# ayumiymk/DiG

Hardware: AMD Instinct MI355X
Metric: pretrain images/sec (32x128, 2-view, mask 0.7) ViT-S/4 (higher is better)
Workload: dtype bf16

## Files before the change

### cpu_abi/dig_cpu.cpp

```cpp
#include <algorithm>
#include <cmath>
#include <cstdint>
#include <cstring>
#include <vector>

typedef void* hipStream_t;
#include "../include/dig_block_types.h"
enum { DIG_OK = 0, DIG_ERR_ARG = -1, DIG_ERR_ALIGN = -2, DIG_ERR_LAUNCH = -3, DIG_ERR_UNSUPPORTED = -4 };
typedef uint16_t bf16_t;

struct dig_dropout_t {
  unsigned k0, k1, thr;
  float scale;
  unsigned pk0, pk1, pthr;
  float pscale;
  int rows_per_sample;
};

namespace {

inline float bf2f(bf16_t h) {
  const uint32_t u = (uint32_t)h << 16;
  float f;
  std::memcpy(&f, &u, 4);
// ... 1009 lines not shown
  for (int k = 0; k < 4; ++k) accs4[k] = stats6[(k >> 1) * 3 + 1 + (k & 1)] * acc_scale;
  return DIG_OK;
}
int dig_step_meters(const float* loss, const float* contra, const float* pixel, const float* accs4, const int* counts, int n_counts,
                    const float* grad_norm, float* out10, hipStream_t) {
  if (!loss || !contra || !pixel || !accs4 || !counts || n_counts <= 0 || !out10) return DIG_ERR_ARG;
  int lo = counts[0], hi = counts[0];
  for (int i = 1; i < n_counts; ++i) { lo = std::min(lo, counts[i]); hi = std::max(hi, counts[i]); }
  out10[0] = loss[0]; out10[1] = contra[0]; out10[2] = pixel[0];
  for (int k = 0; k < 4; ++k) out10[3 + k] = accs4[k];
  out10[7] = (float)lo; out10[8] = (float)hi; out10[9] = grad_norm ? grad_norm[0] : NAN;
  return DIG_OK;
}
int dig_ce_rows(float* logits, int n, int m, int label_offset, float gscale, float* out3, hipStream_t) {
  if (!logits || !out3 || n <= 0 || m <= 0 || label_offset < 0 || label_offset + n > m) return DIG_ERR_ARG;
  for (int i = 0; i < n; ++i) {
    float* row = logits + (size_t)i * m;
    const int label = i + label_offset;
    float mx = -3.0e38f;
    for (int j = 0; j < m; ++j) mx = std::max(mx, row[j]);
    const float zl = row[label];
    float s = 0.f;
    int gt = 0;
    for (int j = 0; j < m; ++j) { s += std::exp(row[j] - mx); gt += row[j] > zl; }
    const float lse = mx + std::log(s);
    for (int j = 0; j < m; ++j) row[j] = gscale * (std::exp(row[j] - mx) / s - (j == label ? 1.f : 0.f));
    out3[0] += lse - zl;
    if (gt < 1) out3[1] += 1.f;
    if (gt < 5) out3[2] += 1.f;
  }
  return DIG_OK;
}

static int adamw_core(float* p, const float* g, float* m, float* v, bf16_t* shadow, long long n, const unsigned char* group, float lr0,
                      float wd0, float lr1, float wd1, float beta1, float beta2, float eps, float inv_bc1, float inv_sqrt_bc2,
                      float grad_scale, const float* finite_gate) {
  if (finite_gate && !std::isfinite(finite_gate[0])) return DIG_OK;
#pragma omp parallel for
  for (long long i = 0; i < n; ++i) {
    const int grp = group[i >> 8] & 0x7f;
    if (grp == 2) {
      if (shadow) shadow[i] = f2bf(p[i]);
      continue;
    }
    const float lr = grp ? lr1 : lr0, wd = grp ? wd1 : wd0;
    const float gk = g[i] * grad_scale;
    float P = p[i] * (1.0f - lr * wd);
    const float M = m[i] * beta1 + gk * (1.0f - beta1);
    const float V = v[i] * beta2 + gk * gk * (1.0f - beta2);
    P -= (lr * inv_bc1) * (M / (std::sqrt(V) * inv_sqrt_bc2 + eps));
    p[i] = P; m[i] = M; v[i] = V;
    if (shadow) shadow[i] = f2bf(P);
  }
  return DIG_OK;
}

int dig_adamw_bias_corrections(float beta1, float beta2, int step, float* out2) {
  if (!out2 || step < 1) return DIG_ERR_ARG;
  out2[0] = (float)(1.0 / (1.0 - std::pow((double)beta1, (double)step)));
  out2[1] = (float)(1.0 / std::sqrt(1.0 - std::pow((double)beta2, (double)step)));
  return DIG_OK;
}

struct AdamTrMat { long long off, dst_off; int rows, cols, tile0, pad; };

int dig_adamw_step_tr(float* p, const float* g, float* m, float* v, void* bf16_shadow, long long n, const unsigned char* group_flags, float lr0,
// ... 557 lines not shown
```

### dig_amd/csrc/loss.hip

```cpp
#include "common.h"

namespace {

__global__ void l2norm_fwd_kernel(const float* __restrict__ x, float* __restrict__ y, float* __restrict__ inv_norm, int n, int C,
                                  float eps) {
  const int r = blockIdx.x * (blockDim.x >> 6) + (threadIdx.x >> 6);
  const int lane = threadIdx.x & 63;
  if (r >= n) return;
  float s = 0.f;
  for (int c = lane; c < C; c += 64) { const float v = x[(size_t)r * C + c]; s += v * v; }
  s = wave_sum(s);
  const float inv = 1.0f / fmaxf(sqrtf(s), eps);
  for (int c = lane; c < C; c += 64) y[(size_t)r * C + c] = x[(size_t)r * C + c] * inv;
  if (lane == 0) inv_norm[r] = inv;
}

__global__ void l2norm_bwd_kernel(const float* __restrict__ dy, const float* __restrict__ y, const float* __restrict__ inv_norm,
                                  float* __restrict__ dx, int n, int C) {
  const int r = blockIdx.x * (blockDim.x >> 6) + (threadIdx.x >> 6);
  const int lane = threadIdx.x & 63;
  if (r >= n) return;
  float s = 0.f;
  for (int c = lane; c < C; c += 64) s += y[(size_t)r * C + c] * dy[(size_t)r * C + c];
  s = wave_sum(s);
  const float inv = inv_norm[r];
  for (int c = lane; c < C; c += 64) dx[(size_t)r * C + c] = (dy[(size_t)r * C + c] - y[(size_t)r * C + c] * s) * inv;
}

template <bool TB>
__global__ __launch_bounds__(256) void sgemm_kernel(const float* __restrict__ A, const float* __restrict__ B, float* __restrict__ C,
                                                    int I, int J, int R, int lda, int ldb, int ldc, float alpha, int r_per_split) {
  constexpr int TS = 32, KS = 64;
  __shared__ float As[KS][TS + 1];
// ... 70 lines not shown
      atomicAdd(out, lse - zl);
      if (gt < 0.5f) atomicAdd(out + 1, 1.f);
      if (gt < 4.5f) atomicAdd(out + 2, 1.f);
    }
    return;
  }
  __shared__ float red2[256];
  const float mine[3] = {lse - zl, gt < 0.5f ? 1.f : 0.f, gt < 4.5f ? 1.f : 0.f};
  float tot[3];
  if (dig_grid_sum_last<3>(ws, mine, tot, red2)) { out[0] += tot[0]; out[1] += tot[1]; out[2] += tot[2]; }
}

__global__ void infonce_finish_kernel(const float* __restrict__ stats6, float loss_scale, float acc_scale, float* __restrict__ contra,
                                      float* __restrict__ accs4) {
  if (threadIdx.x == 0) contra[0] = (stats6[0] + stats6[3]) * loss_scale;
  if (threadIdx.x < 4) accs4[threadIdx.x] = stats6[(threadIdx.x >> 1) * 3 + 1 + (threadIdx.x & 1)] * acc_scale;
}

__global__ __launch_bounds__(64) void step_meters_kernel(const float* __restrict__ loss, const float* __restrict__ contra, const float* __restrict__ pixel,
                                                        const float* __restrict__ accs4, const int* __restrict__ counts, int n_counts,
                                                        const float* __restrict__ grad_norm, float* __restrict__ out10) {
  int lo = 0x7fffffff, hi = -0x7fffffff - 1;
  for (int i = threadIdx.x; i < n_counts; i += 64) { const int c = counts[i]; lo = min(lo, c); hi = max(hi, c); }
#pragma unroll
  for (int o = 32; o > 0; o >>= 1) { lo = min(lo, __shfl_xor(lo, o, 64)); hi = max(hi, __shfl_xor(hi, o, 64)); }
  if (threadIdx.x == 0) {
    out10[0] = loss[0]; out10[1] = contra[0]; out10[2] = pixel[0];
    out10[7] = (float)lo; out10[8] = (float)hi;
    out10[9] = grad_norm ? grad_norm[0] : __builtin_nanf("");
  }
  if (threadIdx.x < 4) out10[3 + threadIdx.x] = accs4[threadIdx.x];
}

}

extern "C" int dig_infonce_finish(const float* stats6, float loss_scale, float acc_scale, float* contra, float* accs4, hipStream_t stream) {
  if (!stats6 || !contra || !accs4) return DIG_ERR_ARG;
  hipLaunchKernelGGL(infonce_finish_kernel, dim3(1), dim3(64), 0, stream, stats6, loss_scale, acc_scale, contra, accs4);
  return dig_check_launch();
}

extern "C" int dig_step_meters(const float* loss, const float* contra, const float* pixel, const float* accs4, const int* counts, int n_counts,
                               const float* grad_norm, float* out10, hipStream_t stream) {
  if (!loss || !contra || !pixel || !accs4 || !counts || n_counts <= 0 || !out10) return DIG_ERR_ARG;
  hipLaunchKernelGGL(step_meters_kernel, dim3(1), dim3(64), 0, stream, loss, contra, pixel, accs4, counts, n_counts, grad_norm, out10);
  return dig_check_launch();
}

extern "C" int dig_l2norm_fwd(const float* x, float* y, float* inv_norm, int n, int C, float eps, hipStream_t stream) {
  if (!x || !y || !inv_norm || n <= 0 || C <= 0) return DIG_ERR_ARG;
  hipLaunchKernelGGL(l2norm_fwd_kernel, dim3((n + 3) / 4), dim3(256), 0, stream, x, y, inv_norm, n, C, eps);
  return dig_check_launch();
}

extern "C" int dig_l2norm_bwd(const float* dy, const float* y, const float* inv_norm, float* dx, int n, int C, hipStream_t stream) {
  if (!dy || !y || !inv_norm || !dx || n <= 0 || C <= 0) return DIG_ERR_ARG;
  hipLaunchKernelGGL(l2norm_bwd_kernel, dim3((n + 3) / 4), dim3(256), 0, stream, dy, y, inv_norm, dx, n, C);
  return dig_check_launch();
}

extern "C" int dig_sgemm(const float* A, const float* B, float* C, int I, int J, int R, int lda, int ldb, int ldc, int trans_b,
                         float alpha, int r_splits, hipStream_t stream) {
  if (!A || !B || !C || I <= 0 || J <= 0 || R <= 0 || r_splits < 1) return DIG_ERR_ARG;
  const int per = ((R + r_splits - 1) / r_splits + 63) / 64 * 64;
  if ((R + per - 1) / per != r_splits) return DIG_ERR_ARG;
  dim3 grid((J + 31) / 32, (I + 31) / 32, r_splits);
  if (trans_b)
    hipLaunchKernelGGL(sgemm_kernel<true>, grid, dim3(256), 0, stream, A, B, C, I, J, R, lda, ldb, ldc, alpha, per);
  else
    hipLaunchKernelGGL(sgemm_kernel<false>, grid, dim3(256), 0, stream, A, B, C, I, J, R, lda, ldb, ldc, alpha, per);
  return dig_check_launch();
}

extern "C" int dig_ce_rows_ws(float* logits, int n, int m, int label_offset, float gscale, float* out3, float* workspace, hipStream_t stream) {
  if (!logits || !out3 || n <= 0 || m <= 0 || label_offset < 0 || label_offset + n > m) return DIG_ERR_ARG;
  hipLaunchKernelGGL(ce_rows_kernel, dim3(n), dim3(256), 0, stream, logits, n, m, label_offset, gscale, out3, workspace);
  return dig_check_launch();
}
extern "C" int dig_ce_rows(float* logits, int n, int m, int label_offset, float gscale, float* out3, hipStream_t stream) {
  return dig_ce_rows_ws(logits, n, m, label_offset, gscale, out3, nullptr, stream);
}
```

### dig_amd/engine_core.py

```python
import ctypes
import functools
import itertools
import os
import weakref
from typing import Optional, Tuple

import torch

from . import block_calls as BC
from . import encoder_blocks as EB
from . import ops
from .parallel import LOCAL, LocalComm, bn_backward, bn_forward

BF16, F32 = torch.bfloat16, torch.float32
FWD_MODE = os.environ.get("DIG_FWD_MODE", "flip")
CHAIN_BWD_EVERY = max(1, int(os.environ.get("DIG_CHAIN_BWD_EVERY", "1")))
CHAIN_BWD_PHASE = int(os.environ.get("DIG_CHAIN_BWD_PHASE", "0"))
BATCH_REDUCE = os.environ.get("DIG_BATCH_REDUCE", "0") == "1"
FUSED_QV_BIAS_SUMS = os.environ.get("DIG_FUSED_QV_BIAS", "1") != "0"
WGRAD_GROUPING = os.environ.get("DIG_WGRAD_GROUPING", "block")
WGRAD_INLINE = os.environ.get("DIG_WGRAD_INLINE", "1") == "1"
WGRAD_DEFER = os.environ.get("DIG_WGRAD_DEFER", "auto").strip().lower()
if WGRAD_DEFER not in ("auto", "0", "1"):
    raise ValueError(f"DIG_WGRAD_DEFER={WGRAD_DEFER!r}: one of auto, 0, 1")
# ... 348 lines not shown
            enc_m, ks = momentum_branch()
            del enc_m
            main.wait_stream(hi_st)
        else:
            side.wait_stream(main)
            with torch.cuda.stream(side):
                enc_m, ks = momentum_branch(heads=not dist_mode)
            enc, self.saved_enc = self.encoder_forward(ew_on, images, aug, mask_u8, True, path=self.path_on)
            self.enc = enc
            if not dist_mode:
                qs = online_heads(enc)
                main.wait_stream(side)
                if side is not main:
                    ks.record_stream(main)
                del enc_m
            else:
                main.wait_stream(side)
                enc_m.record_stream(main)
                if pp:
                    (masked2, self.saved_pix), (masked_m, _) = self.mlp_forward_pair(enc[:B * N], "pix_projector", "online", True,
                                                                                      enc_m[:B * N], "pix_projector_m", "momentum", False)
                else:
                    masked2, self.saved_pix, masked_m = enc[:B * N], None, enc_m[:B * N]
                pooled, self.saved_pnet = extract(masked2, enc, "patch_extractor", "online", True)
                pooled_m, _ = extract(masked_m, enc_m, "momentum_patch_extractor", "momentum", False)
                (qs, self.saved_proj), (ks, _) = self.mlp_forward_pair(pooled, "encoder_projection_layer", "online", True,
                                                                        pooled_m, "momentum_projection_layer", "momentum", False)
                qs, self.saved_pred = self.mlp_forward(qs, "predictor", "online", True)
                del enc_m, masked_m, pooled_m
        _mark("forward: both encoders + heads joined", dev)
        M._flat["bn_count"] += 1
        n = B * M.n_patch
        dim = M.moco_dim
        qf = torch.empty((2 * n, dim), device=dev, dtype=F32)
        kf = torch.empty((2 * n, dim), device=dev, dtype=F32)
        ops.cast_bf16_to_f32(qs, qf)
        ops.cast_bf16_to_f32(ks, kf)
        qn, self.q_inv = ops.l2norm_fwd(qf)
        kn, _ = ops.l2norm_fwd(kf)
        self.qn = qn
        if dist_mode:
            kall = comm.all_gather_cat(kn.view(1, 2, n, dim))
            k1_all = kall[:, 0].reshape(comm.world * n, dim).contiguous()
            k2_all = kall[:, 1].reshape(comm.world * n, dim).contiguous()
        else:
            k1_all, k2_all = kn[:n], kn[n:]
        mk = comm.world * n
        stats = torch.zeros((2, 3), device=dev, dtype=F32)
        self.dqn = torch.empty((2 * n, dim), device=dev, dtype=F32)
        gs = 2.0 * M.T / n
        for half, kk in ((0, k2_all), (1, k1_all)):
            logits = torch.empty((n, mk), device=dev, dtype=F32)
            ops.sgemm(qn[half * n:(half + 1) * n], kk, logits, n, mk, dim, False, 1.0 / M.T)
            ops.ce_rows(logits, n * comm.rank, gs, stats[half])
            ops.sgemm(logits, kk, self.dqn[half * n:(half + 1) * n], n, dim, mk, True, 1.0 / M.T)
        contra, accs = ops.infonce_finish(stats, 2.0 * M.T / n, 100.0 / n)
        if not M.use_pixel_target:
            vis_out = torch.empty((0, 0, M.dec_classes), device=dev, dtype=F32)
            self.mim_views = 0
        elif vis_out is None:
            vis_out, _ = decoder()
        _mark("forward: InfoNCE + SimMIM decoder done", dev)
        return contra, accs, vis_out

    def _decoder_forward(self, mask_u8, images, mim_views):
        M = self.m
        B, N, dev = images.shape[0], M.N, images.device
        per = M._mask_count(mask_u8, B)
        Mrows = mim_views * B * per
        Mp = (Mrows + 63) // 64 * 64
        idx, cnt = ops.mask_to_index(mask_u8[:mim_views * B], per)
        M._last_mask_counts, M._last_idx, M._last_images = cnt, idx[:B], images
        M._last_idx_views = [idx[:B]] + ([(idx[B:] - B * N).clamp_min_(0)] if mim_views == 2 else [])
        self.idx, self.Mrows, self.Mp, self.per, self.mim_views = idx, Mrows, Mp, per, mim_views
        w16, f32 = M._w("online"), M._f32
        gath = ops.gather_rows(self.enc, idx, Mrows, Mp)
        h0 = ops.linear_fwd(gath, w16["pix_decoder.0.weight"])
        h1 = ops.linear_fwd(h0, w16["pix_decoder.1.weight"])
        h2, mu, rs = ops.layernorm_fwd(h1, f32["pix_decoder.2.weight"], f32["pix_decoder.2.bias"], M.ln_eps, gelu=True)
        pred = torch.empty((Mp, 64), device=dev, dtype=F32)
        C = M.dec_classes
        ops.gemm(h2, w16["pix_decoder.4.weight"], Mp, C, M.dec_dim, out=pred, out_kind=ops.OUT_F32, bias=f32["pix_decoder.4.bias"], ldc=64)
        self.saved_dec = (gath, h0, h1, h2, mu, rs)
        return pred[:Mrows, :C].reshape(mim_views * B, per, C)

    def _forward_gen_only(self, ew_on, images, aug, mask_u8, mim_views, training, fresh):
        M = self.m
        dev = images.device
        views = mim_views
        self.gen_views = views
        self.wT = None
        if training and ((ops.mlp_chain_supported(M.D, M.F, views * self.B * M.N) and (ops.MLP_CHAIN_MASK & 4)) or
                         (ops.DGRAD_DIRECT and views * self.B * M.N >= 8192)):
            self.wT = self.mlp_weight_transposes(ew_on, fresh)
        enc_raw, self.saved_enc = self.encoder_forward(ew_on, images, aug, mask_u8, True, views=views, path=self.path_on)
        f32 = M._f32
        self.enc, mu, rs = ops.layernorm_fwd(enc_raw, f32["encoder.norm.weight"], f32["encoder.norm.bias"], M.ln_eps)
        self.saved_norm = (enc_raw, mu, rs)
        vis_out = self._decoder_forward(mask_u8, images, mim_views)
        return torch.zeros((), device=dev, dtype=F32), torch.zeros(4, device=dev, dtype=F32), vis_out

    def backward(self, g_contra, g_vis):
        M = self.m
        B, D, N, nw = self.B, M.D, M.N, M.num_windows
        dev = self.enc.device
        w16, f32, g32 = M._w("online"), M._f32, M._g32
        contrast = g_contra is not None and M.use_moco_target
        if g_vis is not None and not M.use_pixel_target:
            g_vis = None
        self._assign, M._grads_fresh = bool(getattr(M, "_grads_fresh", False)), False
        _mark("backward: start (loss, MSE, autograd entry done)", dev)
        views = 2 if (contrast or (g_vis is not None and self.mim_views == 2)) else 1
        d_enc = torch.empty_like(self.enc) if contrast else torch.zeros((views * B * N, D), device=dev, dtype=BF16)
        n = B * M.n_patch
        if contrast:
            dqn = self.dqn
            ops.scale_by_device_scalar(dqn, g_contra.reshape(1).float())
            dq = ops.l2norm_bwd(dqn, self.qn, self.q_inv)
            dq16 = torch.empty(dq.shape, device=dev, dtype=BF16)
            ops.cast_f32_to_bf16(dq, dq16)
            dproj = self.mlp_backward(dq16, "predictor", self.saved_pred)
            self._grad_ready(dev, "predictor")
            dpool = self.mlp_backward(dproj, "encoder_projection_layer", self.saved_proj)
            self._grad_ready(dev, "encoder_projection_layer")
            acc = False
            if M.patchnet == 'regular':
                from . import patchnet
                dpool, dfeat = patchnet.backward(self, dpool, "patch_extractor", self.saved_pnet, 2 * B)
                self._grad_ready(dev, "patch_extractor")
                d_enc, acc = dfeat, True
            if M.patchnet == 'conv':
                from . import convpatchnet
                d_enc = convpatchnet.backward(self, dpool, "patch_extractor", self.saved_pnet, 2 * B)
                self._grad_ready(dev, "patch_extractor")
                if M.has_pix_projector:
                    self.mlp_backward(d_enc[:B * N], "pix_projector", self.saved_pix, dx_out=d_enc[:B * N])
                    self._grad_ready(dev, "pix_projector")
            elif M.has_pix_projector:
                dmasked2 = d_enc[:B * N] if acc else torch.empty((B * N, D), device=dev, dtype=BF16)
                ops.window_pool_bwd(dpool[:n], dmasked2, B, M.gh, M.gw, nw, D, acc)
                ops.window_pool_bwd(dpool[n:], d_enc[B * N:], B, M.gh, M.gw, nw, D, acc)
                self.mlp_backward(dmasked2, "pix_projector", self.saved_pix, dx_out=d_enc[:B * N])
                self._grad_ready(dev, "pix_projector")
            else:
                ops.window_pool_bwd(dpool[:n], d_enc[:B * N], B, M.gh, M.gw, nw, D, acc)
                ops.window_pool_bwd(dpool[n:], d_enc[B * N:], B, M.gh, M.gw, nw, D, acc)
        elif M.use_moco_target:
            for name in (("predictor", "encoder_projection_layer") + (("patch_extractor",) if M.patchnet != 'no_patchtrans' else ())
                         + (("pix_projector",) if M.has_pix_projector else ())):
                self.comm.grad_ready(M, name)
        if g_vis is not None:
            gath, h0, h1, h2, mu, rs = self.saved_dec
            Mrows, Mp, C, Dd = self.Mrows, self.Mp, M.dec_classes, M.dec_dim
# ... 133 lines not shown
```

### dig_amd/ops.py

```python
import ctypes
import os
from collections import namedtuple

import torch

from . import _lib as L

cf = ctypes.c_float
cll = ctypes.c_longlong
BF16 = torch.bfloat16
F32 = torch.float32

OUT_BF16, OUT_F32, OUT_F32_PARTIAL = 0, 1, 2
GEMM_BK_FWD, GEMM_BK_BWD = 64, 32
_ws = {}


def _stream_id(dev):
    if L._raw_stream is not None and dev.index is not None:
        return L._raw_stream(dev.index)
    return torch.cuda.current_stream(dev).cuda_stream


def _workspace(dev, numel):
# ... 858 lines not shown
SGEMM_SPLIT_SMALL = os.environ.get("DIG_SGEMM_SPLIT_SMALL", "1") != "0"
SGEMM_SPLIT_MIN_R = 256


def sgemm(A, B, C, I, J, R, trans_b, alpha):
    sp = 1
    if R >= 2048 and C.stride(0) == J:
        sp = R // 512
        while sp > 1 and R % (64 * sp):
            sp -= 1
    elif SGEMM_SPLIT_SMALL and R >= SGEMM_SPLIT_MIN_R and I * J <= (1 << 18) and C.stride(0) == J and R % 256 == 0:
        sp = R // 128
    if sp > 1:
        ws = _workspace(A.device, sp * I * J)
        L.call("dig_sgemm", L.ptr(A), L.ptr(B), L.ptr(ws), I, J, R, A.stride(0), B.stride(0), J, int(trans_b), cf(alpha), sp, L.stream())
        L.call("dig_reduce_partials", L.ptr(ws), sp, cll(I * J), L.ptr(C), 0, L.stream())
    else:
        L.call("dig_sgemm", L.ptr(A), L.ptr(B), L.ptr(C), I, J, R, A.stride(0), B.stride(0), C.stride(0), int(trans_b), cf(alpha), 1, L.stream())


def ce_rows(logits, label_offset, gscale, out3):
    n = logits.shape[0]
    L.call("dig_ce_rows_ws", L.ptr(logits), n, logits.shape[1], label_offset, cf(gscale), L.ptr(out3),
           L.ptr(_loss_workspace(logits.device, "ce", 1 + 3 * n)), L.stream())


def infonce_finish(stats, loss_scale, acc_scale):
    contra = torch.empty((), device=stats.device, dtype=F32)
    accs = torch.empty(4, device=stats.device, dtype=F32)
    L.call("dig_infonce_finish", L.ptr(stats), cf(loss_scale), cf(acc_scale), L.ptr(contra), L.ptr(accs), L.stream())
    return contra, accs


def step_meters(loss, contra, pixel, accs4, counts, grad_norm):
    out = torch.empty(10, device=loss.device, dtype=F32)
    L.call("dig_step_meters", L.ptr(loss), L.ptr(contra), L.ptr(pixel), L.ptr(accs4), L.ptr(counts), counts.numel(), L.ptr(grad_norm), L.ptr(out),
           L.stream())
    return out


def cast_f32_to_bf16(x, y, n=None):
    L.call("dig_cast_f32_to_bf16", L.ptr(x), L.ptr(y), cll(x.numel() if n is None else n), L.stream())


def cast_bf16_to_f32(x, y, n=None):
    L.call("dig_cast_bf16_to_f32", L.ptr(x), L.ptr(y), cll(x.numel() if n is None else n), L.stream())


def fill_f32(x, value=0.0):
    L.call("dig_fill_f32", L.ptr(x), cll(x.numel()), cf(value), L.stream())


def scale_f32(x, s):
    L.call("dig_scale_f32", L.ptr(x), cll(x.numel()), cf(s), L.stream())


def scale_by_device_scalar(x, scalar, extra=1.0):
    L.call("dig_scale_by_device_scalar", L.ptr(x), cll(x.numel()), L.ptr(scalar), cf(extra), L.stream())


def pad_cast_rows(src, dst, M, C):
    L.call("dig_pad_cast_rows", L.ptr(src), L.ptr(dst), M, C, dst.shape[0], dst.stride(0), L.stream())


def axpy_f32(y, x, a=1.0):
    L.call("dig_axpy_f32", L.ptr(y), L.ptr(x), cll(x.numel()), cf(a), L.stream())
# ... 36 lines not shown
```

### include/dig_hip.h

```cpp
#ifndef DIG_HIP_H
#define DIG_HIP_H

#ifdef __cplusplus
extern "C" {
#endif

#ifndef __HIP_PLATFORM_AMD__
typedef struct ihipStream_t* hipStream_t;
#endif

#include "dig_aug_types.h"

#define DIG_GEMM_TILE_DEFAULT 0
#define DIG_GEMM_TILE_128x128_K32 32
#define DIG_GEMM_TILE_128x128_K64 64
#define DIG_GEMM_TILE_256x256 244
#define DIG_GEMM_TILE_256x192 264
#define DIG_GEMM_TILE_64x128 212
#define DIG_GEMM_TILE_128x64 221
#define DIG_GEMM_TILE_256x256_PERSISTENT 544
#define DIG_GEMM_TILE_256x192_PERSISTENT 564
int dig_gemm_bf16(const void* A, const void* B, void* C, int I, int J, int R, int lda, int ldb, int ldc, int trans_a,
                  int trans_b, int out_kind, const float* bias, const void* resid, int ldr, void* pre_act, int ldp, float alpha,
                  int alpha_cols, int act, int splits, int a_rows, int b_rows, int bk, float* colsum_partials,
// ... 92 lines not shown
int dig_patch_embed_bwd(const void* dy, const float* img, const unsigned char* mask, float* dW, float* dbias, float* dmask_token,
                        int n_img, int gh, int gw, int D, hipStream_t stream);
int dig_patchify_bf16(const float* img, const unsigned char* mask, void* out, int n_img, int gh, int gw, hipStream_t stream);
int dig_colsum_masked(const void* x, const unsigned char* mask, float* out_unmasked, float* out_masked, float* workspace,
                      int rows, int C, hipStream_t stream);

int dig_window_pool_fwd(const void* x, void* out, int out_is_f32, int n_img, int gh, int gw, int nwin, int D, hipStream_t stream);
int dig_window_pool_bwd(const void* dpool, void* dx, int n_img, int gh, int gw, int nwin, int D, int accumulate, hipStream_t stream);

int dig_im2col3x3(const void* x, void* col, int n_img, int H, int W, int C, int ldc, hipStream_t stream);
int dig_conv3x3_weight_flip(const void* w, void* wt, int c_out, int c_in, hipStream_t stream);
int dig_maxpool2x2_fwd(const void* x, void* y, unsigned char* idx, int n_img, int H, int W, int C, hipStream_t stream);
int dig_maxpool2x2_bwd(const void* dy, const unsigned char* idx, void* dx, int n_img, int H, int W, int C, hipStream_t stream);

int dig_mask_views_u8(const void* mask, int elem_kind, int B, int V, int N, int keep_views, unsigned char* out, hipStream_t stream);
int dig_mask_to_index(const unsigned char* mask, int* idx, int* count, int B, int N, int max_per_sample, hipStream_t stream);
int dig_gather_rows(const void* src, const int* idx, void* dst, int M, int M_pad, int D, hipStream_t stream);
int dig_scatter_rows_add(const void* src, const int* idx, void* dst, int M, int D, hipStream_t stream);
int dig_mim_target(const float* img, const int* idx, float* target, int M, int gh, int gw, int normalize , hipStream_t stream);
int dig_mse_fwd_bwd(const float* pred, int ld_pred, const float* target, int M, int C, float gscale, float* loss, void* dpred,
                    int ld_dpred, hipStream_t stream);

int dig_l2norm_fwd(const float* x, float* y, float* inv_norm, int n, int C, float eps, hipStream_t stream);
int dig_l2norm_bwd(const float* dy, const float* y, const float* inv_norm, float* dx, int n, int C, hipStream_t stream);
int dig_sgemm(const float* A, const float* B, float* C, int I, int J, int R, int lda, int ldb, int ldc, int trans_b, float alpha,
              int r_splits , hipStream_t stream);
int dig_ce_rows(float* logits, int n, int m, int label_offset, float gscale, float* out3, hipStream_t stream);
int dig_mse_fwd_bwd_ws(const float* pred, int ld_pred, const float* target, int M, int C, float gscale, float* loss, void* dpred,
                       int ld_dpred, float* workspace, hipStream_t stream);
int dig_ce_rows_ws(float* logits, int n, int m, int label_offset, float gscale, float* out3, float* workspace, hipStream_t stream);
int dig_infonce_finish(const float* stats6, float loss_scale, float acc_scale, float* contra, float* accs4, hipStream_t stream);
int dig_step_meters(const float* loss, const float* contra, const float* pixel, const float* accs4, const int* counts, int n_counts,
                    const float* grad_norm, float* out10, hipStream_t stream);

int dig_adamw_step(float* p, const float* g, float* m, float* v, void* bf16_shadow, long long n, const unsigned char* group_flags,
                   float lr0, float wd0, float lr1, float wd1, float beta1, float beta2, float eps, int step, float grad_scale,
                   const float* finite_gate, hipStream_t stream);
int dig_adamw_step_tr(float* p, const float* g, float* m, float* v, void* bf16_shadow, long long n, const unsigned char* group_flags,
                      float lr0, float wd0, float lr1, float wd1, float beta1, float beta2, float eps, int step, float grad_scale,
                      const float* finite_gate, const void* mats, int n_mats, int n_tiles, void* tr_out, hipStream_t stream);
int dig_adamw_step_groups(float* p, const float* g, float* m, float* v, void* bf16_shadow, long long n, const unsigned char* group_idx,
                          const float* lr_tab, const float* wd_tab, float beta1, float beta2, float eps, int step, float grad_scale,
                          const float* finite_gate, hipStream_t stream);
int dig_ema_update(float* pm, const float* p, void* bf16_shadow, long long n, float m, hipStream_t stream);
int dig_adamw_bias_corrections(float beta1, float beta2, int step, float* out2_host);
int dig_adamw_step_dev(float* p, const float* g, float* m, float* v, void* bf16_shadow, long long n, const unsigned char* group_flags,
                       const float* scalars6, float beta1, float beta2, float eps, float grad_scale, const float* finite_gate,
                       hipStream_t stream);
int dig_ema_update_dev(float* pm, const float* p, void* bf16_shadow, long long n, const float* m_and_one_minus_m, hipStream_t stream);
long long dig_sumsq_workspace_bytes(long long n);
int dig_sumsq(const float* x, long long n, float* workspace, float* out, hipStream_t stream);

long long dig_colsum_workspace_bytes(int rows, int C);
int dig_colsum(const void* x, float* out, float* workspace, int rows, int C, int ld, hipStream_t stream);
int dig_colsum_partials(const float* partials, int n_parts, int C, float* out, hipStream_t stream);
#define DIG_COLSUM_MAX_SEGS 112
typedef struct dig_colsum_seg { const float* partials; float* out; long long stride; int n_parts; int C; } dig_colsum_seg_t;
int dig_colsum_partials_multi(const dig_colsum_seg_t* segs, int n_segs, hipStream_t stream);
int dig_gelu_bwd(const void* dact, const void* pre, void* dpre, long long n, hipStream_t stream);
int dig_add_bf16(const void* a, const void* b, void* out, long long n, hipStream_t stream);
int dig_cast_f32_to_bf16(const float* x, void* y, long long n, hipStream_t stream);
int dig_cast_bf16_to_f32(const void* x, float* y, long long n, hipStream_t stream);
int dig_pad_cast_rows(const float* src, void* dst, int M, int C, int M_pad, int ld, hipStream_t stream);
int dig_fill_f32(float* x, long long n, float value, hipStream_t stream);
int dig_scale_f32(float* x, long long n, float s, hipStream_t stream);
int dig_scale_by_device_scalar(float* x, long long n, const float* scalar, float extra, hipStream_t stream);
// ... 118 lines not shown
```

Measured before the change: 6721.

## Fuse InfoNCE logits, cross-entropy and dq GEMM into one LDS-resident kernel

Adds a fused kernel that computes q·k logits, the softmax cross-entropy gradient and the dq back-projection per 8-row block, with the logits kept in LDS instead of going through global memory. It also fuses the bf16 cast with l2norm forward for q and k, and fuses the scale, l2norm backward and bf16 cast in the backward pass. The aim is to cut kernel launches and global memory round-trips for the small contrastive head. The trade-off is low parallelism (few blocks), scalar fp32 dot products, and a large LDS footprint. An sgemm fallback with split-K reduction is kept for shapes that do not fit.

Result: no change. 6752 (median of 6 runs) (+0.5%).

```diff
diff --git a/cpu_abi/dig_cpu.cpp b/cpu_abi/dig_cpu.cpp
--- a/cpu_abi/dig_cpu.cpp
+++ b/cpu_abi/dig_cpu.cpp
@@ -1065,6 +1065,55 @@
   return DIG_OK;
 }
 
+int dig_cast_bf16_to_f32(const void* x, float* y, long long n, hipStream_t);
+int dig_cast_f32_to_bf16(const float* x, void* y, long long n, hipStream_t);
+int dig_scale_by_device_scalar(float* x, long long n, const float* scalar, float extra, hipStream_t);
+int dig_cast_l2norm_rows(const void* xa, float* ya, float* inv_a, int na, const void* xb, float* yb, float* inv_b, int nb, int C, float eps,
+                         hipStream_t st) {
+  if (!xa || !ya || na <= 0 || nb < 0 || C <= 0 || (nb > 0 && (!xb || !yb))) return DIG_ERR_ARG;
+  for (int set = 0; set < (nb > 0 ? 2 : 1); ++set) {
+    const bf16_t* x = (const bf16_t*)(set ? xb : xa);
+    float* y = set ? yb : ya;
+    float* inv = set ? inv_b : inv_a;
+    const int n = set ? nb : na;
+    std::vector<float> xf((size_t)n * C), iv(n);
+    for (size_t i = 0; i < xf.size(); ++i) xf[i] = bf2f(x[i]);
+    const int rc = dig_l2norm_fwd(xf.data(), y, iv.data(), n, C, eps, st);
+    if (rc != DIG_OK) return rc;
+    if (inv) std::copy(iv.begin(), iv.end(), inv);
+  }
+  return DIG_OK;
+}
+
+int dig_l2norm_bwd_scaled_bf16(const float* dy, const float* g, const float* y, const float* inv_norm, void* dx, int n, int C, hipStream_t st) {
+  if (!dy || !g || !y || !inv_norm || !dx || n <= 0 || C <= 0) return DIG_ERR_ARG;
+  std::vector<float> d(dy, dy + (size_t)n * C), o((size_t)n * C);
+  int rc = dig_scale_by_device_scalar(d.data(), (long long)d.size(), g, 1.0f, st);
+  if (rc == DIG_OK) rc = dig_l2norm_bwd(d.data(), y, inv_norm, o.data(), n, C, st);
+  if (rc != DIG_OK) return rc;
+  for (size_t i = 0; i < o.size(); ++i) ((bf16_t*)dx)[i] = f2bf(o[i]);
+  return DIG_OK;
+}
+
+long long dig_infonce_workspace_floats(int n, int mk, int C) { return (n <= 0 || mk <= 0 || C <= 0) ? 0 : 6LL * n; }
+
+int dig_infonce_fwd_bwd(const float* qn, const float* k_half0, const float* k_half1, float* dqn, float* contra, float* accs4, float* workspace,
+                        int n, int mk, int C, int label_offset, float inv_T, float gscale, float loss_scale, float acc_scale, int, hipStream_t st) {
+  if (!qn || !k_half0 || !k_half1 || !dqn || !contra || !accs4 || !workspace || n <= 0 || mk <= 0 || C <= 0 || (C & 3) || label_offset < 0 ||
+      label_offset + n > mk)
+    return DIG_ERR_ARG;
+  std::vector<float> logits((size_t)n * mk);
+  float stats[6] = {0.f, 0.f, 0.f, 0.f, 0.f, 0.f};
+  for (int half = 0; half < 2; ++half) {
+    const float* k = half ? k_half1 : k_half0;
+    int rc = dig_sgemm(qn + (size_t)half * n * C, k, logits.data(), n, mk, C, C, C, mk, 0, inv_T, 1, st);
+    if (rc == DIG_OK) rc = dig_ce_rows(logits.data(), n, mk, label_offset, gscale, stats + 3 * half, st);
+    if (rc == DIG_OK) rc = dig_sgemm(logits.data(), k, dqn + (size_t)half * n * C, n, C, mk, mk, C, C, 1, inv_T, 1, st);
+    if (rc != DIG_OK) return rc;
+  }
+  return dig_infonce_finish(stats, loss_scale, acc_scale, contra, accs4, st);
+}
+
 static int adamw_core(float* p, const float* g, float* m, float* v, bf16_t* shadow, long long n, const unsigned char* group, float lr0,
                       float wd0, float lr1, float wd1, float beta1, float beta2, float eps, float inv_bc1, float inv_sqrt_bc2,
                       float grad_scale, const float* finite_gate) {
diff --git a/dig_amd/csrc/loss.hip b/dig_amd/csrc/loss.hip
--- a/dig_amd/csrc/loss.hip
+++ b/dig_amd/csrc/loss.hip
@@ -1,4 +1,6 @@
 #include "common.h"
+
+extern "C" int dig_reduce_partials(const float* partials, int splits, long long n, float* out, int accumulate, hipStream_t stream);
 
 namespace {
 
@@ -135,6 +137,178 @@
   if (threadIdx.x < 4) out10[3 + threadIdx.x] = accs4[threadIdx.x];
 }
 
+__global__ void cast_l2norm_rows_kernel(const bf16_t* __restrict__ xa, float* __restrict__ ya, float* __restrict__ inva, int na,
+                                        const bf16_t* __restrict__ xb, float* __restrict__ yb, float* __restrict__ invb, int nb, int C,
+                                        float eps) {
+  int r = blockIdx.x * (blockDim.x >> 6) + (threadIdx.x >> 6);
+  const int lane = threadIdx.x & 63;
+  if (r >= na + nb) return;
+  const bf16_t* x = xa;
+  float* y = ya;
+  float* inv_norm = inva;
+  if (r >= na) { r -= na; x = xb; y = yb; inv_norm = invb; }
+  float s = 0.f;
+  for (int c = lane; c < C; c += 64) { const float v = bf2f(x[(size_t)r * C + c]); s += v * v; }
+  s = wave_sum(s);
+  const float inv = 1.0f / fmaxf(sqrtf(s), eps);
+  for (int c = lane; c < C; c += 64) y[(size_t)r * C + c] = bf2f(x[(size_t)r * C + c]) * inv;
+  if (lane == 0 && inv_norm) inv_norm[r] = inv;
+}
+
+__global__ void l2norm_bwd_scaled_bf16_kernel(const float* __restrict__ dy, const float* __restrict__ gptr, const float* __restrict__ y,
+                                              const float* __restrict__ inv_norm, bf16_t* __restrict__ dx, int n, int C) {
+  const int r = blockIdx.x * (blockDim.x >> 6) + (threadIdx.x >> 6);
+  const int lane = threadIdx.x & 63;
+  if (r >= n) return;
+  const float g = gptr[0];
+  float s = 0.f;
+  for (int c = lane; c < C; c += 64) {
+    float d = dy[(size_t)r * C + c] * g;
+    asm volatile("" : "+v"(d));
+    s += y[(size_t)r * C + c] * d;
+  }
+  s = wave_sum(s);
+  const float inv = inv_norm[r];
+  for (int c = lane; c < C; c += 64) {
+    float d = dy[(size_t)r * C + c] * g;
+    asm volatile("" : "+v"(d));
+    dx[(size_t)r * C + c] = f2bf((d - y[(size_t)r * C + c] * s) * inv);
+  }
+}
+
+constexpr int NCE_RB = 8, NCE_KT = 256, NCE_KS = 32, NCE_KP = NCE_KS + 4;
+
+__global__ __launch_bounds__(256) void infonce_fused_kernel(const float* __restrict__ qn, const float* __restrict__ k_half0,
+                                                            const float* __restrict__ k_half1, float* __restrict__ dqn,
+                                                            float* __restrict__ rows3, int n, int mk, int mkp, int C, int label_offset,
+                                                            float inv_T, float gscale) {
+  extern __shared__ __align__(16) float nce_lds[];
+  float* qs = nce_lds;
+  float* Ks = qs + NCE_RB * C;
+  float* lg = Ks + NCE_KT * NCE_KP;
+  const int nblk = (n + NCE_RB - 1) / NCE_RB;
+  const int half = blockIdx.x / nblk, r0 = (blockIdx.x - half * nblk) * NCE_RB;
+  const float* __restrict__ k = half ? k_half1 : k_half0;
+  const float* __restrict__ q = qn + (size_t)half * n * C;
+  const int tid = threadIdx.x;
+  const int C4 = C >> 2;
+  for (int e = tid; e < NCE_RB * C4; e += 256) {
+    const int r = e / C4, c4 = e - r * C4;
+    float4 v = make_float4(0.f, 0.f, 0.f, 0.f);
+    if (r0 + r < n) v = reinterpret_cast<const float4*>(q + (size_t)(r0 + r) * C)[c4];
+    reinterpret_cast<float4*>(qs)[e] = v;
+  }
+  for (int j0 = 0; j0 < mk; j0 += NCE_KT) {
+    float acc[NCE_RB];
+#pragma unroll
+    for (int r = 0; r < NCE_RB; ++r) acc[r] = 0.f;
+    for (int d0 = 0; d0 < C; d0 += NCE_KS) {
+      __syncthreads();
+      for (int e = tid; e < NCE_KT * NCE_KS / 4; e += 256) {
+        const int jj = e >> 3, d4 = e & 7;
+        float4 v = make_float4(0.f, 0.f, 0.f, 0.f);
+        if (j0 + jj < mk) v = *reinterpret_cast<const float4*>(k + (size_t)(j0 + jj) * C + d0 + d4 * 4);
+        *reinterpret_cast<float4*>(Ks + jj * NCE_KP + d4 * 4) = v;
+      }
+      __syncthreads();
+#pragma unroll
+      for (int d4 = 0; d4 < NCE_KS / 4; ++d4) {
+        const float4 kv = *reinterpret_cast<const float4*>(Ks + tid * NCE_KP + d4 * 4);
+#pragma unroll
+        for (int r = 0; r < NCE_RB; ++r) {
+          const float4 qv = *reinterpret_cast<const float4*>(qs + r * C + d0 + d4 * 4);
+          acc[r] += qv.x * kv.x; acc[r] += qv.y * kv.y; acc[r] += qv.z * kv.z; acc[r] += qv.w * kv.w;
+        }
+      }
+    }
+    if (j0 + tid < mk) {
+#pragma unroll
+      for (int r = 0; r < NCE_RB; ++r) lg[r * mkp + j0 + tid] = acc[r] * inv_T;
+    }
+  }
+  __syncthreads();
+  const int lane = tid & 63, wv = tid >> 6;
+  for (int rr = wv; rr < NCE_RB; rr += 4) {
+    float* row = lg + rr * mkp;
+    const int gi = r0 + rr;
+    if (lane < mkp - mk) row[mk + lane] = 0.f;
+    if (gi >= n) continue;
+    const int label = gi + label_offset;
+    float mx = -3.0e38f;
+    for (int j = lane; j < mk; j += 64) mx = fmaxf(mx, row[j]);
+    mx = wave_max(mx);
+    const float zl = row[label];
+    float s = 0.f, gt = 0.f;
+    for (int j = lane; j < mk; j += 64) {
+      const float z = row[j];
+      s += __expf(z - mx);
+      gt += (z > zl) ? 1.f : 0.f;
+    }
+    s = wave_sum(s);
+    gt = wave_sum(gt);
+    const float lse = mx + __logf(s);
+    const float inv = 1.0f / s;
+    for (int j = lane; j < mk; j += 64) {
+      const float p = __expf(row[j] - mx) * inv;
+      row[j] = gscale * (p - (j == label ? 1.f : 0.f));
+    }
+    if (lane == 0) {
+      float* o = rows3 + ((size_t)half * n + gi) * 3;
+      o[0] = lse - zl; o[1] = gt < 0.5f ? 1.f : 0.f; o[2] = gt < 4.5f ? 1.f : 0.f;
+    }
+  }
+  __syncthreads();
+  const int mk4 = mk & ~3;
+  for (int c = tid; c < C; c += 256) {
+    float acc[NCE_RB];
+#pragma unroll
+    for (int r = 0; r < NCE_RB; ++r) acc[r] = 0.f;
+#pragma unroll 2
+    for (int j = 0; j < mk4; j += 4) {
+      const float k0 = k[(size_t)j * C + c], k1 = k[(size_t)(j + 1) * C + c], k2 = k[(size_t)(j + 2) * C + c], k3 = k[(size_t)(j + 3) * C + c];
+#pragma unroll
+      for (int r = 0; r < NCE_RB; ++r) {
+        const float4 g = *reinterpret_cast<const float4*>(lg + r * mkp + j);
+        acc[r] += g.x * k0; acc[r] += g.y * k1; acc[r] += g.z * k2; acc[r] += g.w * k3;
+      }
+    }
+    for (int j = mk4; j < mk; ++j) {
+      const float kv = k[(size_t)j * C + c];
+#pragma unroll
+      for (int r = 0; r < NCE_RB; ++r) acc[r] += lg[r * mkp + j] * kv;
+    }
+#pragma unroll
+    for (int r = 0; r < NCE_RB; ++r)
+      if (r0 + r < n) dqn[((size_t)half * n + r0 + r) * C + c] = acc[r] * inv_T;
+  }
+}
+
+__global__ __launch_bounds__(256) void infonce_finish_rows_kernel(const float* __restrict__ rows3, int n, float loss_scale, float acc_scale,
+                                                                  float* __restrict__ contra, float* __restrict__ accs4) {
+  __shared__ float red[4 * 6];
+  float a[6];
+#pragma unroll
+  for (int v = 0; v < 6; ++v) a[v] = 0.f;
+  for (int i = threadIdx.x; i < n; i += 256) {
+#pragma unroll
+    for (int v = 0; v < 3; ++v) { a[v] += rows3[(size_t)i * 3 + v]; a[3 + v] += rows3[((size_t)n + i) * 3 + v]; }
+  }
+#pragma unroll
+  for (int v = 0; v < 6; ++v) {
+    a[v] = wave_sum(a[v]);
+    if ((threadIdx.x & 63) == 0) red[(threadIdx.x >> 6) * 6 + v] = a[v];
+  }
+  __syncthreads();
+  if (threadIdx.x < 6) {
+    float t = 0.f;
+    for (int w = 0; w < 4; ++w) t += red[w * 6 + threadIdx.x];
+    red[threadIdx.x] = t;
+  }
+  __syncthreads();
+  if (threadIdx.x == 0) contra[0] = (red[0] + red[3]) * loss_scale;
+  if (threadIdx.x < 4) accs4[threadIdx.x] = red[(threadIdx.x >> 1) * 3 + 1 + (threadIdx.x & 1)] * acc_scale;
+}
+
 }
 
 extern "C" int dig_infonce_finish(const float* stats6, float loss_scale, float acc_scale, float* contra, float* accs4, hipStream_t stream) {
@@ -183,3 +357,72 @@
 extern "C" int dig_ce_rows(float* logits, int n, int m, int label_offset, float gscale, float* out3, hipStream_t stream) {
   return dig_ce_rows_ws(logits, n, m, label_offset, gscale, out3, nullptr, stream);
 }
+
+extern "C" int dig_cast_l2norm_rows(const void* xa, float* ya, float* inv_a, int na, const void* xb, float* yb, float* inv_b, int nb, int C,
+                                    float eps, hipStream_t stream) {
+  if (!xa || !ya || na <= 0 || nb < 0 || C <= 0 || (nb > 0 && (!xb || !yb))) return DIG_ERR_ARG;
+  hipLaunchKernelGGL(cast_l2norm_rows_kernel, dim3((na + nb + 3) / 4), dim3(256), 0, stream, (const bf16_t*)xa, ya, inv_a, na, (const bf16_t*)xb,
+                     yb, inv_b, nb, C, eps);
+  return dig_check_launch();
+}
+
+extern "C" int dig_l2norm_bwd_scaled_bf16(const float* dy, const float* g, const float* y, const float* inv_norm, void* dx, int n, int C,
+                                          hipStream_t stream) {
+  if (!dy || !g || !y || !inv_norm || !dx || n <= 0 || C <= 0) return DIG_ERR_ARG;
+  hipLaunchKernelGGL(l2norm_bwd_scaled_bf16_kernel, dim3((n + 3) / 4), dim3(256), 0, stream, dy, g, y, inv_norm, (bf16_t*)dx, n, C);
+  return dig_check_launch();
+}
+
+static size_t nce_lds_bytes(int mk, int C) { return ((size_t)NCE_RB * C + (size_t)NCE_KT * NCE_KP + (size_t)NCE_RB * ((mk + 3) & ~3)) * sizeof(float); }
+static bool nce_resident(int mk, int C) { return C % NCE_KS == 0 && C <= 1024 && mk <= 2048 && nce_lds_bytes(mk, C) <= 160 * 1024; }
+static int nce_dq_splits(int mk) {
+  int sp = mk >= 2048 ? mk / 512 : 1;
+  while (sp > 1 && mk % (64 * sp)) --sp;
+  return sp;
+}
+
+extern "C" long long dig_infonce_workspace_floats(int n, int mk, int C) {
+  if (n <= 0 || mk <= 0 || C <= 0) return 0;
+  const long long head = 8 + ((1 + 3LL * n + 3) & ~3LL);
+  return std::max<long long>(6LL * n, head + (((long long)n * mk + 3) & ~3LL) + (long long)nce_dq_splits(mk) * n * C);
+}
+
+extern "C" int dig_infonce_fwd_bwd(const float* qn, const float* k_half0, const float* k_half1, float* dqn, float* contra, float* accs4,
+                                   float* workspace, int n, int mk, int C, int label_offset, float inv_T, float gscale, float loss_scale,
+                                   float acc_scale, int resident, hipStream_t stream) {
+  if (!qn || !k_half0 || !k_half1 || !dqn || !contra || !accs4 || !workspace || n <= 0 || mk <= 0 || C <= 0 || (C & 3) || label_offset < 0 ||
+      label_offset + n > mk)
+    return DIG_ERR_ARG;
+  if (!aligned16(qn) || !aligned16(k_half0) || !aligned16(k_half1) || !aligned16(workspace)) return DIG_ERR_ALIGN;
+  if (resident && nce_resident(mk, C)) {
+    const int lds = (int)nce_lds_bytes(mk, C);
+    static int attr_lds[DIG_MAX_DEVICES] = {};
+    const int dev = dig_device();
+    if (lds > attr_lds[dev]) {
+      if (hipFuncSetAttribute(reinterpret_cast<const void*>(infonce_fused_kernel), hipFuncAttributeMaxDynamicSharedMemorySize, lds) != hipSuccess)
+        return DIG_ERR_LAUNCH;
+      attr_lds[dev] = lds;
+    }
+    hipLaunchKernelGGL(infonce_fused_kernel, dim3(2 * ((n + NCE_RB - 1) / NCE_RB)), dim3(256), lds, stream, qn, k_half0, k_half1, dqn, workspace,
+                       n, mk, (mk + 3) & ~3, C, label_offset, inv_T, gscale);
+    hipLaunchKernelGGL(infonce_finish_rows_kernel, dim3(1), dim3(256), 0, stream, workspace, n, loss_scale, acc_scale, contra, accs4);
+    return dig_check_launch();
+  }
+  const long long head = 8 + ((1 + 3LL * n + 3) & ~3LL);
+  float* stats = workspace;
+  float* ce_ws = workspace + 8;
+  float* logits = workspace + head;
+  float* slabs = logits + (((long long)n * mk + 3) & ~3LL);
+  const int sp = ((long long)n * C) % 4 == 0 ? nce_dq_splits(mk) : 1;
+  if (hipMemsetAsync(workspace, 0, head * sizeof(float), stream) != hipSuccess) return DIG_ERR_LAUNCH;
+  for (int half = 0; half < 2; ++half) {
+    const float* k = half ? k_half1 : k_half0;
+    float* dq = dqn + (size_t)half * n * C;
+    int rc = dig_sgemm(qn + (size_t)half * n * C, k, logits, n, mk, C, C, C, mk, 0, inv_T, 1, stream);
+    if (rc == DIG_OK) rc = dig_ce_rows_ws(logits, n, mk, label_offset, gscale, stats + 3 * half, ce_ws, stream);
+    if (rc == DIG_OK) rc = dig_sgemm(logits, k, sp > 1 ? slabs : dq, n, C, mk, mk, C, C, 1, inv_T, sp, stream);
+    if (rc == DIG_OK && sp > 1) rc = dig_reduce_partials(slabs, sp, (long long)n * C, dq, 0, stream);
+    if (rc != DIG_OK) return rc;
+  }
+  return dig_infonce_finish(stats, loss_scale, acc_scale, contra, accs4, stream);
+}
diff --git a/dig_amd/engine_core.py b/dig_amd/engine_core.py
--- a/dig_amd/engine_core.py
+++ b/dig_amd/engine_core.py
@@ -404,12 +404,16 @@
         M._flat["bn_count"] += 1
         n = B * M.n_patch
         dim = M.moco_dim
-        qf = torch.empty((2 * n, dim), device=dev, dtype=F32)
-        kf = torch.empty((2 * n, dim), device=dev, dtype=F32)
-        ops.cast_bf16_to_f32(qs, qf)
-        ops.cast_bf16_to_f32(ks, kf)
-        qn, self.q_inv = ops.l2norm_fwd(qf)
-        kn, _ = ops.l2norm_fwd(kf)
+        fused = ops.INFONCE_FUSED
+        if fused:
+            qn, self.q_inv, kn = ops.cast_l2norm_rows(qs, ks)
+        else:
+            qf = torch.empty((2 * n, dim), device=dev, dtype=F32)
+            kf = torch.empty((2 * n, dim), device=dev, dtype=F32)
+            ops.cast_bf16_to_f32(qs, qf)
+            ops.cast_bf16_to_f32(ks, kf)
+            qn, self.q_inv = ops.l2norm_fwd(qf)
+            kn, _ = ops.l2norm_fwd(kf)
         self.qn = qn
         if dist_mode:
             kall = comm.all_gather_cat(kn.view(1, 2, n, dim))
@@ -418,15 +422,18 @@
         else:
             k1_all, k2_all = kn[:n], kn[n:]
         mk = comm.world * n
-        stats = torch.zeros((2, 3), device=dev, dtype=F32)
-        self.dqn = torch.empty((2 * n, dim), device=dev, dtype=F32)
-        gs = 2.0 * M.T / n
-        for half, kk in ((0, k2_all), (1, k1_all)):
-            logits = torch.empty((n, mk), device=dev, dtype=F32)
-            ops.sgemm(qn[half * n:(half + 1) * n], kk, logits, n, mk, dim, False, 1.0 / M.T)
-            ops.ce_rows(logits, n * comm.rank, gs, stats[half])
-            ops.sgemm(logits, kk, self.dqn[half * n:(half + 1) * n], n, dim, mk, True, 1.0 / M.T)
-        contra, accs = ops.infonce_finish(stats, 2.0 * M.T / n, 100.0 / n)
+        if fused:
+            self.dqn, contra, accs = ops.infonce_fwd_bwd(qn, k2_all, k1_all, n, n * comm.rank, M.T)
+        else:
+            stats = torch.zeros((2, 3), device=dev, dtype=F32)
+            self.dqn = torch.empty((2 * n, dim), device=dev, dtype=F32)
+            gs = 2.0 * M.T / n
+            for half, kk in ((0, k2_all), (1, k1_all)):
+                logits = torch.empty((n, mk), device=dev, dtype=F32)
+                ops.sgemm(qn[half * n:(half + 1) * n], kk, logits, n, mk, dim, False, 1.0 / M.T)
+                ops.ce_rows(logits, n * comm.rank, gs, stats[half])
+                ops.sgemm(logits, kk, self.dqn[half * n:(half + 1) * n], n, dim, mk, True, 1.0 / M.T)
+            contra, accs = ops.infonce_finish(stats, 2.0 * M.T / n, 100.0 / n)
         if not M.use_pixel_target:
             vis_out = torch.empty((0, 0, M.dec_classes), device=dev, dtype=F32)
             self.mim_views = 0
@@ -487,10 +494,16 @@
         n = B * M.n_patch
         if contrast:
             dqn = self.dqn
-            ops.scale_by_device_scalar(dqn, g_contra.reshape(1).float())
-            dq = ops.l2norm_bwd(dqn, self.qn, self.q_inv)
-            dq16 = torch.empty(dq.shape, device=dev, dtype=BF16)
-            ops.cast_f32_to_bf16(dq, dq16)
+            g1 = g_contra.reshape(1)
+            if g1.dtype != F32:
+                g1 = g1.float()
+            if ops.L2BWD_FUSED:
+                dq16 = ops.l2norm_bwd_scaled_bf16(dqn, g1, self.qn, self.q_inv)
+            else:
+                ops.scale_by_device_scalar(dqn, g1)
+                dq = ops.l2norm_bwd(dqn, self.qn, self.q_inv)
+                dq16 = torch.empty(dq.shape, device=dev, dtype=BF16)
+                ops.cast_f32_to_bf16(dq, dq16)
             dproj = self.mlp_backward(dq16, "predictor", self.saved_pred)
             self._grad_ready(dev, "predictor")
             dpool = self.mlp_backward(dproj, "encoder_projection_layer", self.saved_proj)
diff --git a/dig_amd/ops.py b/dig_amd/ops.py
--- a/dig_amd/ops.py
+++ b/dig_amd/ops.py
@@ -914,6 +914,39 @@
     return contra, accs
 
 
+INFONCE_FUSED = os.environ.get("DIG_INFONCE_FUSED", "1") != "0"
+L2BWD_FUSED = os.environ.get("DIG_L2BWD_FUSED", "1") != "0"
+
+
+def cast_l2norm_rows(xa, xb=None, eps=1e-12):
+    C = xa.shape[1]
+    ya = torch.empty(xa.shape, device=xa.device, dtype=F32)
+    inv = torch.empty(xa.shape[0], device=xa.device, dtype=F32)
+    yb = torch.empty(xb.shape, device=xa.device, dtype=F32) if xb is not None else None
+    L.call("dig_cast_l2norm_rows", L.ptr(xa), L.ptr(ya), L.ptr(inv), xa.shape[0], L.ptr(xb), L.ptr(yb), None, xb.shape[0] if xb is not None else 0,
+           C, cf(eps), L.stream())
+    return ya, inv, yb
+
+
+def infonce_fwd_bwd(qn, k_half0, k_half1, n, label_offset, T, resident=True):
+    mk, C = k_half0.shape
+    f = L.lib().dig_infonce_workspace_floats
+    f.restype = ctypes.c_longlong
+    ws = _workspace2(qn.device, int(f(n, mk, C)))
+    dqn = torch.empty((2 * n, C), device=qn.device, dtype=F32)
+    contra = torch.empty((), device=qn.device, dtype=F32)
+    accs = torch.empty(4, device=qn.device, dtype=F32)
+    L.call("dig_infonce_fwd_bwd", L.ptr(qn), L.ptr(k_half0), L.ptr(k_half1), L.ptr(dqn), L.ptr(contra), L.ptr(accs), L.ptr(ws), n, mk, C,
+           label_offset, cf(1.0 / T), cf(2.0 * T / n), cf(2.0 * T / n), cf(100.0 / n), int(resident), L.stream())
+    return dqn, contra, accs
+
+
+def l2norm_bwd_scaled_bf16(dy, g, y, inv):
+    dx = torch.empty(y.shape, device=y.device, dtype=BF16)
+    L.call("dig_l2norm_bwd_scaled_bf16", L.ptr(dy), L.ptr(g), L.ptr(y), L.ptr(inv), L.ptr(dx), y.shape[0], y.shape[1], L.stream())
+    return dx
+
+
 def step_meters(loss, contra, pixel, accs4, counts, grad_norm):
     out = torch.empty(10, device=loss.device, dtype=F32)
     L.call("dig_step_meters", L.ptr(loss), L.ptr(contra), L.ptr(pixel), L.ptr(accs4), L.ptr(counts), counts.numel(), L.ptr(grad_norm), L.ptr(out),
diff --git a/include/dig_hip.h b/include/dig_hip.h
--- a/include/dig_hip.h
+++ b/include/dig_hip.h
@@ -148,6 +148,14 @@
 int dig_infonce_finish(const float* stats6, float loss_scale, float acc_scale, float* contra, float* accs4, hipStream_t stream);
 int dig_step_meters(const float* loss, const float* contra, const float* pixel, const float* accs4, const int* counts, int n_counts,
                     const float* grad_norm, float* out10, hipStream_t stream);
+int dig_cast_l2norm_rows(const void* xa, float* ya, float* inv_a, int na, const void* xb, float* yb, float* inv_b, int nb, int C, float eps,
+                         hipStream_t stream);
+long long dig_infonce_workspace_floats(int n, int mk, int C);
+int dig_infonce_fwd_bwd(const float* qn, const float* k_half0, const float* k_half1, float* dqn, float* contra, float* accs4,
+                        float* workspace, int n, int mk, int C, int label_offset, float inv_T, float gscale, float loss_scale,
+                        float acc_scale, int resident, hipStream_t stream);
+int dig_l2norm_bwd_scaled_bf16(const float* dy, const float* g, const float* y, const float* inv_norm, void* dx, int n, int C,
+                               hipStream_t stream);
 
 int dig_adamw_step(float* p, const float* g, float* m, float* v, void* bf16_shadow, long long n, const unsigned char* group_flags,
                    float lr0, float wd0, float lr1, float wd1, float beta1, float beta2, float eps, int step, float grad_scale,
```
